# seung-lab/igneous

Hardware: NVIDIA H100
Metric: Mvoxels/s on 2048x2048x1024 uint32 seg per GPU (downsample+CCL+mesh) @1/2/4/8 H100; % HBM roofline (higher is better)
Workload: dtype u32

## Files before the change

### igneous_b200/csrc/simplify.cu

```cuda
#include <cub/device/device_radix_sort.cuh>
#include <cub/device/device_scan.cuh>

#include <stdlib.h>

#include <algorithm>
#include <type_traits>

#include "mesher.h"

namespace ign {

constexpr uint64_t S_KEYMAX = 0xFFFFFFFFFFFFFFFFull;
constexpr int S_MAXV = 32;
constexpr int S_VCAP = 64;
constexpr int VB = 11;

struct Simp {
  uint64_t U, T;
  double* pos;
  double* Q;
  uint32_t* face;
  uint32_t* flabel;
  uint8_t* falive;
  uint8_t* valive;
// ... 10 lines not shown
__device__ __forceinline__ uint32_t s_unmix(uint32_t x) {
  x ^= x >> 16; x *= 0x43021123U; x ^= x >> 15 ^ x >> 30; x *= 0x1d69e2a5U; x ^= x >> 16;
  return x;
}
__device__ __forceinline__ uint32_t s_mix16(uint32_t x) {
  x &= 0xFFFFu;
  x = (x * 0x2F35u) & 0xFFFFu; x ^= x >> 7;
  x = (x * 0x4A6Bu) & 0xFFFFu; x ^= x >> 9;
  x = (x * 0x9E37u) & 0xFFFFu; x ^= x >> 8;
  return x;
}
__device__ __forceinline__ uint32_t s_unmix16(uint32_t x) {
  x &= 0xFFFFu;
  x ^= x >> 8; x = (x * 0x7787u) & 0xFFFFu;
  x ^= x >> 9; x = (x * 0x1243u) & 0xFFFFu;
  x ^= x >> 7; x ^= x >> 14; x = (x * 0xEB1Du) & 0xFFFFu;
  return x;
}
__device__ __forceinline__ unsigned long long s_key(double cost, uint32_t h, uint32_t salt) {
  const float c = __double2float_rn(cost);
  return ((unsigned long long)__float_as_uint(c) << 32) | s_mix(h ^ salt);
}

__device__ __forceinline__ double s_qeval(const double* q, const double* p) {
  const double x = p[0], y = p[1], z = p[2];
  return q[0] * x * x + 2.0 * q[1] * x * y + 2.0 * q[2] * x * z + 2.0 * q[3] * x + q[4] * y * y +
         2.0 * q[5] * y * z + 2.0 * q[6] * y + q[7] * z * z + 2.0 * q[8] * z + q[9];
}

__device__ int s_twins(const Simp& s, uint32_t f, uint32_t u, uint32_t v, uint32_t* twin) {
  int cnt = 0;
  const uint32_t* lu = s.vf + (uint64_t)u * S_VCAP;
  const uint32_t cu = s.vn[u];
  for (uint32_t j = 0; j < cu; j++) {
    const uint32_t h = lu[j];
    const uint32_t g = h / 3;
    if (g == f || !s.falive[g]) continue;
    const uint32_t* fv = s.face + 3 * (uint64_t)g;
    if (fv[0] == v || fv[1] == v || fv[2] == v) {
      if (cnt == 0) *twin = h;
      cnt++;
    }
  }
  return cnt;
}

struct SEval {
  bool valid;
  double cost;
  uint32_t keep, remove;
  double p[3];
};

__device__ __forceinline__ void s_cost(const double* Q, const double* pos, double max_err2, uint32_t u, uint32_t v,
                                       uint64_t gu, uint64_t gv, bool bu, bool bv, SEval* e) {
  e->valid = false;
  if (bu && bv) return;
  const double* Qu = Q + 10 * gu;
  const double* Qv = Q + 10 * gv;
  double q[10];
#pragma unroll
  for (int i = 0; i < 10; i++) q[i] = Qu[i] + Qv[i];
  const double* pu = pos + 3 * gu;
  const double* pv = pos + 3 * gv;
  double best[3], cost;
  if (bu) {
    e->keep = u;
    e->remove = v;
    best[0] = pu[0]; best[1] = pu[1]; best[2] = pu[2];
    cost = s_qeval(q, best);
  } else if (bv) {
    e->keep = v;
    e->remove = u;
    best[0] = pv[0]; best[1] = pv[1]; best[2] = pv[2];
    cost = s_qeval(q, best);
  } else {
    e->keep = u < v ? u : v;
    e->remove = u < v ? v : u;
    const double* pk = u < v ? pu : pv;
    const double* pr = u < v ? pv : pu;
    const double kk[3] = {pk[0], pk[1], pk[2]}, rr[3] = {pr[0], pr[1], pr[2]};
    const double mid[3] = {(kk[0] + rr[0]) * 0.5, (kk[1] + rr[1]) * 0.5, (kk[2] + rr[2]) * 0.5};
    const double ck = s_qeval(q, kk), cr = s_qeval(q, rr), cm = s_qeval(q, mid);
    cost = ck;
    best[0] = kk[0]; best[1] = kk[1]; best[2] = kk[2];
    if (cr < cost) { cost = cr; best[0] = rr[0]; best[1] = rr[1]; best[2] = rr[2]; }
    if (cm < cost) { cost = cm; best[0] = mid[0]; best[1] = mid[1]; best[2] = mid[2]; }
  }
  if (cost < 0.0) cost = 0.0;
  if (!(cost <= max_err2)) return;
  e->valid = true;
  e->cost = cost;
  e->p[0] = best[0]; e->p[1] = best[1]; e->p[2] = best[2];
}

__global__ void __launch_bounds__(256)
    k_simp_init_verts(const uint64_t* __restrict__ vkeys, uint64_t U, double rx, double ry, double rz,
                      double* __restrict__ pos, uint8_t* __restrict__ valive,
                      uint8_t* __restrict__ vbound, uint32_t* __restrict__ vn) {
  const uint64_t i = blockIdx.x * (uint64_t)blockDim.x + threadIdx.x;
  if (i >= U) return;
  const uint64_t k = vkeys[i];
  const double x = (double)(k & ((1u << VB) - 1));
  const double y = (double)((k >> VB) & ((1u << VB) - 1));
  const double z = (double)((k >> (2 * VB)) & ((1u << VB) - 1));
  pos[3 * i + 0] = x * 0.5 * rx;
  pos[3 * i + 1] = y * 0.5 * ry;
  pos[3 * i + 2] = z * 0.5 * rz;
  valive[i] = 1;
  vbound[i] = 0;
  vn[i] = 0;
}

__global__ void __launch_bounds__(256)
    k_simp_init_faces(const uint32_t* __restrict__ faces_local, const uint32_t* __restrict__ tri_off,
                      const uint32_t* __restrict__ vert_off, uint32_t K, uint64_t T,
                      uint32_t* __restrict__ face, uint32_t* __restrict__ flabel,
                      uint8_t* __restrict__ falive, uint32_t* __restrict__ node_vertex,
                      uint32_t* __restrict__ node_id) {
  const uint64_t f = blockIdx.x * (uint64_t)blockDim.x + threadIdx.x;
  if (f >= T) return;
  uint32_t lo = 1, hi = K;
  while (lo < hi) {
    const uint32_t mid = (lo + hi + 1) >> 1;
    if (tri_off[mid] <= f) lo = mid;
    else hi = mid - 1;
  }
  flabel[f] = lo;
  falive[f] = 1;
  for (int k = 0; k < 3; k++) {
    const uint32_t g = faces_local[3 * f + k] + vert_off[lo];
    face[3 * f + k] = g;
    node_vertex[3 * f + k] = g;
    node_id[3 * f + k] = (uint32_t)(3 * f + k);
  }
}

__global__ void __launch_bounds__(256)
    k_simp_link(const uint32_t* __restrict__ sv, const uint32_t* __restrict__ sh, uint64_t n,
                uint32_t* __restrict__ vf, uint32_t* __restrict__ vn, uint32_t* overflow) {
  const uint64_t i = blockIdx.x * (uint64_t)blockDim.x + threadIdx.x;
  if (i >= n) return;
  const uint32_t v = sv[i];
  if (i > 0 && sv[i - 1] == v) return;
  uint32_t c = 0;
  for (uint64_t j = i; j < n && sv[j] == v; j++) {
// ... 109 lines not shown
__host__ __device__ inline bool sl_fits_smem(uint32_t T, uint32_t U, uint32_t threads, size_t smem_bytes,
                                             bool resumed = false) {
  const uint32_t cap = (uint32_t)SL_LIST_PER * threads;
  return 3ull * T <= 65536ull && T <= cap && U <= cap && sl_layout(T, U, resumed).need <= smem_bytes;
}
__host__ __device__ inline uint32_t sl_wcap(uint32_t T, uint32_t U, uint32_t threads, size_t smem_bytes,
                                            bool resumed, uint32_t limit) {
  const size_t w = SL_WCAP + (smem_bytes - sl_layout(T, U, resumed).need) / SL_WIN_BYTES;
  const size_t m = threads < limit ? threads : limit;
  return (uint32_t)(w < m ? w : m);
}

struct SlArgs {
  double* pos;
  double* Q;
  uint32_t* face;
  uint8_t* falive;
  uint8_t* valive;
  const uint8_t* vbound;
  float* ecost;
  unsigned long long* key1;
  uint8_t* fstate;
  uint8_t* vflag;
  uint8_t* vlose;
  uint32_t *flist, *flist2;
  uint32_t *vlist, *vlist2;
  const uint32_t* tri_off;
  const uint32_t* vert_off;
  const uint32_t* target;
  const uint32_t* order;
  uint32_t K;
  uint32_t base;
  uint32_t cls;
  uint32_t* counters;
  double max_err2;
  int max_rounds;
  uint32_t smem_bytes;
  uint32_t* mq_next;
  uint32_t smem_next;
  const uint32_t* mq;
  uint16_t* finv;
  int persist;
  uint32_t* lrec;
  uint32_t* trace;
  uint32_t wcap_max;
  uint32_t group_min;
};

constexpr int SL_HIST = 1664, SL_HP = 16, SL_HW = 64, SL_HR = S_MAXV + 2, SL_HCLS = SL_HP + SL_HW + SL_HR;

constexpr int SL_MREC = 8;
constexpr int SL_LREC = 7;
constexpr int SL_NPH = 9;

struct SlShared {
  uint32_t work, alive, progress, ncol, nwin, stop, slow, counter, npass;
  uint32_t ring8, ring16;
  uint32_t nnarrow, nwide;
  uint32_t rec, valive;
  unsigned long long visits, wins;
  long long t_label;
  uint32_t nrecost;
  uint32_t ngroup[3];
  unsigned long long ph[SL_NPH];
  long long t_prev;
};

template <bool SM>
struct SlLab {
  typedef typename std::conditional<SM, uint16_t, uint32_t>::type idx_t;
  uint32_t T, U, tbase, vbase, target, label;
  idx_t *fc0, *fc1, *fc2;
  idx_t *fmap, *vmap;
  uint32_t* gface;
  uint8_t* fstate;
  uint8_t* vflag;
  uint8_t* vlose;
  typedef typename std::conditional<SM, uint32_t, unsigned long long>::type key_t;
  key_t* key1;
  bool fmt16;
  uint32_t wcap;
  idx_t* ring;
  idx_t *flist, *flist2, *vlist, *vlist2;
};

template <bool SM>
__device__ __forceinline__ uint32_t sl_fget(const SlLab<SM>& L, uint32_t f, int c) {
  if (SM) return c == 0 ? L.fc0[f] : (c == 1 ? L.fc1[f] : L.fc2[f]);
  return L.gface[3 * (uint64_t)f + c] - L.vbase;
}
template <bool SM>
__device__ __forceinline__ void sl_fset(const SlLab<SM>& L, uint32_t f, int c, uint32_t x) {
  typedef typename SlLab<SM>::idx_t idx_t;
  if (SM) {
    if (c == 0) L.fc0[f] = (idx_t)x;
    else if (c == 1) L.fc1[f] = (idx_t)x;
    else L.fc2[f] = (idx_t)x;
  } else {
    L.gface[3 * (uint64_t)f + c] = x + L.vbase;
  }
}
template <bool SM, bool R>
__device__ __forceinline__ uint64_t sl_vg(const SlLab<SM>& L, uint32_t v) {
  return L.vbase + (uint64_t)(R ? (uint32_t)L.vmap[v] : v);
}
template <bool SM, bool R>
// ... 4 lines not shown
__device__ __forceinline__ void sl_vor(uint8_t* vflag, uint32_t v, uint32_t bits) {
  const uintptr_t a = (uintptr_t)(vflag + v);
  if ((*(volatile uint8_t*)a & bits) == bits) return;
  const uint32_t word = bits << (8 * (a & 3));
  if (SM) {
    asm volatile("red.shared.or.b32 [%0], %1;" ::"r"((uint32_t)__cvta_generic_to_shared((void*)(a & ~(uintptr_t)3))), "r"(word) : "memory");
  } else {
    atomicOr((uint32_t*)(a & ~(uintptr_t)3), word);
  }
}
template <bool SM>
__device__ __forceinline__ void sl_vclear(uint8_t* vflag, uint32_t v, uint32_t bits) {
  const uintptr_t a = (uintptr_t)(vflag + v);
  const uint32_t word = ~(bits << (8 * (a & 3)));
  if (SM) {
    asm volatile("red.shared.and.b32 [%0], %1;" ::"r"((uint32_t)__cvta_generic_to_shared((void*)(a & ~(uintptr_t)3))), "r"(word) : "memory");
  } else {
    atomicAnd((uint32_t*)(a & ~(uintptr_t)3), word);
  }
}
__device__ __forceinline__ void sl_post(unsigned long long* key1, uint32_t u, uint32_t v, unsigned long long key) {
  if (key < *(volatile unsigned long long*)&key1[u]) atomicMin(&key1[u], key);
  if (key < *(volatile unsigned long long*)&key1[v]) atomicMin(&key1[v], key);
}
__device__ __forceinline__ void sl_post(uint32_t* key1, uint32_t u, uint32_t v, uint32_t key) {
  if (key < *(volatile uint32_t*)&key1[u])
    asm volatile("red.shared.min.u32 [%0], %1;" ::"r"((uint32_t)__cvta_generic_to_shared(key1 + u)), "r"(key) : "memory");
  if (key < *(volatile uint32_t*)&key1[v])
    asm volatile("red.shared.min.u32 [%0], %1;" ::"r"((uint32_t)__cvta_generic_to_shared(key1 + v)), "r"(key) : "memory");
}
template <bool SM>
__device__ __forceinline__ typename SlLab<SM>::key_t sl_key(const SlLab<SM>& L, float cost, uint32_t hl, uint32_t salt) {
  typedef typename SlLab<SM>::key_t key_t;
  const uint32_t bits = __float_as_uint(cost);
  if (SM || L.fmt16) return (key_t)((((bits >> 15) & 0xFFFFu) << 16) | s_mix16((hl ^ salt) & 0xFFFFu));
  return (key_t)(((unsigned long long)bits << 32) | s_mix(hl ^ salt));
}
template <bool SM>
__device__ __forceinline__ uint32_t sl_key_edge(const SlLab<SM>& L, typename SlLab<SM>::key_t key, uint32_t salt) {
  if (SM || L.fmt16) return s_unmix16((uint32_t)key & 0xFFFFu) ^ (salt & 0xFFFFu);
  return s_unmix((uint32_t)((unsigned long long)key & 0xFFFFFFFFull)) ^ salt;
}

template <bool SM, bool R>
__device__ __forceinline__ void sl_cost(const SlArgs& A, const SlLab<SM>& L, uint32_t u, uint32_t v, SEval* e) {
  s_cost(A.Q, A.pos, A.max_err2, u, v, sl_vg<SM, R>(L, u), sl_vg<SM, R>(L, v), (L.vflag[u] & VF_BOUND) != 0,
         (L.vflag[v] & VF_BOUND) != 0, e);
}

template <bool SM>
__device__ __forceinline__ uint32_t sl_kcorner(const SlLab<SM>& L, uint32_t f, uint32_t k) {
  return sl_fget<SM>(L, f, 0) == k ? 0u : (sl_fget<SM>(L, f, 1) == k ? 1u : 2u);
}
template <bool SM, bool R>
__device__ __forceinline__ uint32_t sl_recost(const SlArgs& A, const SlLab<SM>& L, uint32_t f, uint32_t c) {
  const uint32_t u = sl_fget<SM>(L, f, (int)c), v = sl_fget<SM>(L, f, (int)((c + 1) % 3));
  SEval ev;
  sl_cost<SM, R>(A, L, u, v, &ev);
  if (!ev.valid) return 3;
  A.ecost[3 * (uint64_t)(L.tbase + sl_fo<SM, R>(L, f)) + c] = __double2float_rn(ev.cost);
  return 2;
}

template <bool SM, bool R>
__device__ __forceinline__ bool sl_flips(const SlArgs& A, const SlLab<SM>& L, const uint32_t* a, uint32_t w,
                                         const double* best) {
  double P[3][3], N[3][3];
#pragma unroll
  for (int k = 0; k < 3; k++) {
    const double* p = A.pos + 3 * sl_vg<SM, R>(L, a[k]);
    P[k][0] = p[0]; P[k][1] = p[1]; P[k][2] = p[2];
  }
#pragma unroll
  for (int k = 0; k < 3; k++) {
    const bool mv = (a[k] == w);
    N[k][0] = mv ? best[0] : P[k][0];
    N[k][1] = mv ? best[1] : P[k][1];
    N[k][2] = mv ? best[2] : P[k][2];
  }
  const double ax = P[1][0] - P[0][0], ay = P[1][1] - P[0][1], az = P[1][2] - P[0][2];
  const double bx = P[2][0] - P[0][0], by = P[2][1] - P[0][1], bz = P[2][2] - P[0][2];
  const double n0x = ay * bz - az * by, n0y = az * bx - ax * bz, n0z = ax * by - ay * bx;
  const double cx = N[1][0] - N[0][0], cy = N[1][1] - N[0][1], cz = N[1][2] - N[0][2];
  const double dx = N[2][0] - N[0][0], dy = N[2][1] - N[0][1], dz = N[2][2] - N[0][2];
  const double n1x = cy * dz - cz * dy, n1y = cz * dx - cx * dz, n1z = cx * dy - cy * dx;
  const double dot = n0x * n1x + n0y * n1y + n0z * n1z;
  return !(dot > 0.0);
}

__device__ __forceinline__ void sl_others(const uint32_t* a, uint32_t w, uint32_t* o1, uint32_t* o2) {
  if (a[0] == w) { *o1 = a[1]; *o2 = a[2]; }
  else if (a[1] == w) { *o1 = a[2]; *o2 = a[0]; }
  else { *o1 = a[0]; *o2 = a[1]; }
}

__device__ __forceinline__ uint32_t sl_distinct(uint32_t x1, uint32_t x2, uint32_t n, uint32_t lane, bool* f1,
                                                bool* f2) {
  const uint32_t FULL = 0xFFFFFFFFu;
  const bool have = lane < n;
  const uint32_t m1 = __match_any_sync(FULL, x1);
  const uint32_t m2 = __match_any_sync(FULL, x2);
  *f1 = have && ((int)lane == __ffs(m1) - 1);
  bool in1 = false;
  for (uint32_t j = 0; j < n; j++) in1 |= (__shfl_sync(FULL, x1, j) == x2);
  *f2 = have && ((int)lane == __ffs(m2) - 1) && !in1;
  return __popc(__ballot_sync(FULL, *f1)) + __popc(__ballot_sync(FULL, *f2));
}

template <bool SM, typename IDX, typename PRED>
__device__ __forceinline__ uint32_t sl_compact(IDX*& list, IDX*& list2, uint32_t n, uint32_t* counter, PRED alive) {
  const uint32_t FULL = 0xFFFFFFFFu;
// ... 25 lines not shown
    if (lane == 31 && inc) base = atomicAdd(counter, inc);
    base = __shfl_sync(FULL, base, 31) + inc - cnt;
#pragma unroll
    for (int k = 0; k < SL_LIST_PER; k++)
      if ((m >> k) & 1u) list[base++] = keep[k];
  } else {
    for (uint32_t i0 = (tid & ~31u); i0 < n; i0 += blockDim.x) {
      const uint32_t i = i0 + lane;
      IDX e = 0;
      bool al = false;
      if (i < n) {
        e = list[i];
        al = alive((uint32_t)e);
      }
      const uint32_t bal = __ballot_sync(FULL, al);
      if (!bal) continue;
      uint32_t base = 0;
      const int leader = __ffs(bal) - 1;
      if ((int)lane == leader) base = atomicAdd(counter, (uint32_t)__popc(bal));
      base = __shfl_sync(FULL, base, leader);
      if (al) list2[base + __popc(bal & ((1u << lane) - 1u))] = e;
    }
    IDX* t = list;
    list = list2;
    list2 = t;
  }
  __syncthreads();
  const uint32_t kept = *counter;
  __syncthreads();
  return kept;
}

#define SL_MARK(id)                                   \
  do {                                                \
    if (A.trace != nullptr && tid == 0) {             \
      const long long _t = clock64();                 \
      sh.ph[id] += (unsigned long long)(_t - sh.t_prev); \
      sh.t_prev = _t;                                 \
    }                                                 \
  } while (0)

extern __shared__ __align__(16) unsigned char sl_smem[];

__device__ __forceinline__ SlWin* sl_win() { return (SlWin*)sl_smem; }

__device__ __forceinline__ uint32_t sl_width(uint32_t nfu, uint32_t nfv, uint32_t wmin) {
  const uint32_t n = nfu > nfv ? nfu : nfv;
  const uint32_t w = n <= 8u ? 8u : (n <= 16u ? 16u : 32u);
  return w > wmin ? w : wmin;
}

template <bool SM, bool R, int W>
__device__ __forceinline__ void sl_group_pass(const SlArgs& A, const SlLab<SM>& L, SlShared& sh, uint32_t first,
                                              uint32_t last, uint32_t* nev) {
  static_assert(W == 8 || W == 16 || W == 32, "group width");
  const uint32_t FULL = 0xFFFFFFFFu;
  const uint32_t tid = threadIdx.x, lane = tid & 31u, warp = tid >> 5, NW = blockDim.x >> 5;
  constexpr uint32_t G = 32 / W;
  const uint32_t gl = lane & (W - 1), goff = lane & ~(uint32_t)(W - 1);
  const uint32_t wmask = W == 32 ? FULL : (1u << W) - 1u;
  const uint32_t gmask = wmask << goff;
  const uint32_t gidx = lane / W;
  SlWin* const win = sl_win();
  for (uint32_t base = first + warp * G; base < last; base += NW * G) {
    bool act = base + gidx < last;
    uint32_t slot = 0, nfu = 0, nfv = 0;
    if (act) {
      slot = win[base + gidx].order;
      nfu = win[slot].cnt[0]; nfv = win[slot].cnt[1];
    }
    act = act && sl_width(nfu, nfv, A.group_min) == (uint32_t)W;
    const uint32_t b_act = __ballot_sync(FULL, act && gl == 0);
    if (!b_act) continue;
    if (lane == 0) atomicAdd(&sh.ngroup[W == 8 ? 0 : (W == 16 ? 1 : 2)], (uint32_t)__popc(b_act));
    if (W == 32 && act && gl == 0 && (nfu > (uint32_t)S_MAXV || nfv > (uint32_t)S_MAXV)) atomicAdd(&A.counters[25], 1u);
    uint32_t fu = 0, fv = 0, u = 0, v = 0, hl = 0, k = 0;
    bool ok = false;
    if (act) {
      if (gl < nfu) fu = L.ring[(2 * slot) * S_MAXV + gl];
      if (gl < nfv) fv = L.ring[(2 * slot + 1) * S_MAXV + gl];
      u = win[slot].u; v = win[slot].v; hl = win[slot].h; k = win[slot].keep;
      ok = !(win[slot].flags & WF_BAD) && nfu <= (uint32_t)S_MAXV && nfv <= (uint32_t)S_MAXV;
    }
    uint32_t au[3] = {0, 0, 0}, av[3] = {0, 0, 0};
    if (ok && gl < nfu) { au[0] = sl_fget<SM>(L, fu, 0); au[1] = sl_fget<SM>(L, fu, 1); au[2] = sl_fget<SM>(L, fu, 2); }
    if (ok && gl < nfv) { av[0] = sl_fget<SM>(L, fv, 0); av[1] = sl_fget<SM>(L, fv, 1); av[2] = sl_fget<SM>(L, fv, 2); }
    {
      bool flip = false;
      if (ok && gl < nfu && au[0] != v && au[1] != v && au[2] != v) flip = sl_flips<SM, R>(A, L, au, u, win[slot].best);
      if (ok && gl < nfv && av[0] != u && av[1] != u && av[2] != u) flip |= sl_flips<SM, R>(A, L, av, v, win[slot].best);
      if (__ballot_sync(FULL, flip) & gmask) ok = false;
    }
    const uint32_t rm = (k == u) ? v : u;
    const uint64_t gk = sl_vg<SM, R>(L, k), gr = sl_vg<SM, R>(L, rm);
    double* Qk = A.Q + 10 * gk;
    const double* Qr = A.Q + 10 * gr;
    double qk = 0.0, qr = 0.0, qk2 = 0.0, qr2 = 0.0;
    if (ok && gl < 10) { qk = Qk[gl]; qr = Qr[gl]; }
    if (W == 8 && ok && gl < 2) { qk2 = Qk[gl + 8]; qr2 = Qr[gl + 8]; }
    const bool hu = ok && gl < nfu, hv = ok && gl < nfv;
    uint32_t x1 = 0xF0000000u + lane, x2 = 0xF1000000u + lane, y1 = 0xF2000000u + lane, y2 = 0xF3000000u + lane;
    if (hu) sl_others(au, u, &x1, &x2);
    if (hv) sl_others(av, v, &y1, &y2);
    const uint32_t nu = ok ? nfu : 0u, nv = ok ? nfv : 0u;
    uint32_t nmax = nu > nv ? nu : nv;
#pragma unroll
    for (uint32_t d = W; d < 32u; d <<= 1) {
      const uint32_t o = __shfl_xor_sync(FULL, nmax, d);
      nmax = o > nmax ? o : nmax;
    }
    const uint32_t mu1 = __match_any_sync(FULL, x1) & gmask, mu2 = __match_any_sync(FULL, x2) & gmask;
    const uint32_t mv1 = __match_any_sync(FULL, y1) & gmask, mv2 = __match_any_sync(FULL, y2) & gmask;
    bool inu = false, inv = false, c1 = false, c2 = false;
    for (uint32_t j = 0; j < nmax; j++) {
      const uint32_t sx1 = __shfl_sync(FULL, x1, j, W), sy1 = __shfl_sync(FULL, y1, j, W), sy2 = __shfl_sync(FULL, y2, j, W);
      if (j < nu) inu |= (sx1 == x2);
      if (j < nv) {
        inv |= (sy1 == y2);
        c1 |= (x1 == sy1) | (x1 == sy2);
        c2 |= (x2 == sy1) | (x2 == sy2);
      }
    }
    const bool f1 = hu && ((int)lane == __ffs(mu1) - 1);
    const bool f2 = hu && ((int)lane == __ffs(mu2) - 1) && !inu;
    const bool g1 = hv && ((int)lane == __ffs(mv1) - 1);
    const bool g2 = hv && ((int)lane == __ffs(mv2) - 1) && !inv;
    const uint32_t b_f1 = __ballot_sync(FULL, f1), b_f2 = __ballot_sync(FULL, f2);
    const uint32_t b_g1 = __ballot_sync(FULL, g1), b_g2 = __ballot_sync(FULL, g2);
    const uint32_t b_c1 = __ballot_sync(FULL, f1 && c1), b_c2 = __ballot_sync(FULL, f2 && c2);
    const uint32_t b_sh = __ballot_sync(FULL, hu && (x1 == v || x2 == v));
    const uint32_t nnu = __popc(b_f1 & gmask) + __popc(b_f2 & gmask), nnv = __popc(b_g1 & gmask) + __popc(b_g2 & gmask);
    const uint32_t common = __popc(b_c1 & gmask) + __popc(b_c2 & gmask), shared = __popc(b_sh & gmask);
    const bool go = ok && nnu <= (uint32_t)S_MAXV && nnv <= (uint32_t)S_MAXV && shared == 2 && common == 2;
    if (act && !go && gl == 0) {
      const uint32_t f = hl / 3, c = hl - 3 * f;
      const uint32_t st = L.fstate[f];
      L.fstate[f] = (uint8_t)((st & ~(3u << (2 * c))) | (1u << (2 * c)));
      sl_vclear<SM>(L.vflag, u, VF_END);
      sl_vclear<SM>(L.vflag, v, VF_END);
      atomicOr(&sh.progress, 1u);
    }
    const bool rm_is_u = (rm == u);
    const bool hr = go && (rm_is_u ? hu : hv);
    const uint32_t rf = rm_is_u ? fu : fv;
    const uint32_t r0 = rm_is_u ? au[0] : av[0], r1 = rm_is_u ? au[1] : av[1], r2 = rm_is_u ? au[2] : av[2];
    const bool dies = hr && (r0 == k || r1 == k || r2 == k);
    if (hr) {
      if (dies) L.fstate[rf] = (uint8_t)(L.fstate[rf] & 0x7Fu);
      else sl_fset<SM>(L, rf, r0 == rm ? 0 : (r1 == rm ? 1 : 2), k);
    }
    const uint32_t dead = __popc(__ballot_sync(FULL, dies) & gmask);
    if (go) {
      if (hu && x1 != v && x2 != v) { sl_vor<SM>(L.vflag, x1, VF_RDIRTY); sl_vor<SM>(L.vflag, x2, VF_RDIRTY); }
      if (hv && y1 != u && y2 != u) { sl_vor<SM>(L.vflag, y1, VF_RDIRTY); sl_vor<SM>(L.vflag, y2, VF_RDIRTY); }
      if (gl < 10) Qk[gl] = qk + qr;
      if (gl >= 10 && gl < 13) A.pos[3 * gk + (gl - 10)] = win[slot].best[gl - 10];
      if (W == 8) {
        if (gl < 2) Qk[gl + 8] = qk2 + qr2;
        else if (gl < 5) A.pos[3 * gk + (gl - 2)] = win[slot].best[gl - 2];
      }
      if (gl == 0) {
        sl_vclear<SM>(L.vflag, k, VF_END);
        sl_vclear<SM>(L.vflag, rm, 0xFFu);
        atomicSub(&sh.alive, dead);
        atomicAdd(&sh.ncol, 1u);
        atomicOr(&sh.progress, 1u);
      }
    }
    __syncwarp();
    uint32_t m = 0, ck = 0, st0 = 0, st1 = 0;
    if (go && gl < nfu) {
      st0 = L.fstate[fu];
      if (st0 & 0x80u) {
        const uint32_t c = sl_kcorner<SM>(L, fu, k);
        ck = c;
        m |= (k < sl_fget<SM>(L, fu, (int)((c + 1) % 3)) ? 1u : 0u) | (sl_fget<SM>(L, fu, (int)((c + 2) % 3)) < k ? 2u : 0u);
      }
    }
    if (go && gl < nfv) {
      st1 = L.fstate[fv];
      if (st1 & 0x80u) {
        const uint32_t c = sl_kcorner<SM>(L, fv, k);
        ck |= c << 2;
        m |= (k < sl_fget<SM>(L, fv, (int)((c + 1) % 3)) ? 4u : 0u) | (sl_fget<SM>(L, fv, (int)((c + 2) % 3)) < k ? 8u : 0u);
      }
    }
    const uint32_t cnt = __popc(m);
    uint32_t inc = cnt;
#pragma unroll
    for (uint32_t d = 1; d < W; d <<= 1) {
      const uint32_t o = __shfl_up_sync(FULL, inc, d, W);
      if (gl >= d) inc += o;
    }
    const uint32_t P = inc - cnt, N = __shfl_sync(FULL, inc, W - 1, W);
    uint32_t rounds = (N + W - 1) / W;
#pragma unroll
    for (uint32_t d = W; d < 32u; d <<= 1) {
      const uint32_t o = __shfl_xor_sync(FULL, rounds, d);
      rounds = o > rounds ? o : rounds;
    }
    uint32_t res = 0;
    for (uint32_t r = 0; r < rounds; r++) {
      const uint32_t idx = r * W + gl;
      uint32_t own = 0;
      for (uint32_t j = 1; j < W; j++)
        if (__shfl_sync(FULL, P, j, W) <= idx) own = j;
      const uint32_t mo = __shfl_sync(FULL, m, own, W), po = __shfl_sync(FULL, P, own, W);
      const uint32_t fuo = __shfl_sync(FULL, fu, own, W), fvo = __shfl_sync(FULL, fv, own, W);
      const uint32_t cko = __shfl_sync(FULL, ck, own, W);
      if (idx < N) {
        uint32_t b = mo;
        for (uint32_t q = idx - po; q; q--) b &= b - 1;
        const uint32_t bit = (uint32_t)__ffs(b) - 1, side = bit >> 1;
        const uint32_t c = (((cko >> (2 * side)) & 3u) + 2u * (bit & 1u)) % 3u;
        res |= sl_recost<SM, R>(A, L, side ? fvo : fuo, c) << (2 * r);
        (*nev)++;
      }
    }
    uint32_t q = P;
#pragma unroll
    for (uint32_t bit = 0; bit < 4; bit++) {
      const uint32_t val = __shfl_sync(FULL, res, q % W, W);
      if ((m >> bit) & 1u) {
        const uint32_t side = bit >> 1, es = (val >> (2 * (q / W))) & 3u;
        const uint32_t c = (((ck >> (2 * side)) & 3u) + 2u * (bit & 1u)) % 3u;
        if (side) st1 = (st1 & ~(3u << (2 * c))) | (es << (2 * c));
        else st0 = (st0 & ~(3u << (2 * c))) | (es << (2 * c));
        q++;
      }
    }
    if (m & 3u) L.fstate[fu] = (uint8_t)st0;
    if (m & 12u) L.fstate[fv] = (uint8_t)st1;
  }
}

template <bool R>
__device__ void sl_migrate(const SlArgs& A, const SlLab<true>& L, SlShared& sh, const uint16_t* flist, uint32_t nF,
                           int r) {
  const uint32_t FULL = 0xFFFFFFFFu;
  const uint32_t tid = threadIdx.x, NT = blockDim.x, lane = tid & 31u, warp = tid >> 5, NW = NT >> 5;
  uint32_t* const wsum = (uint32_t*)sl_win();
  const uint32_t per = (L.U + NT - 1) / NT, v0 = min(tid * per, L.U), v1 = min(v0 + per, L.U);
  uint32_t cnt = 0;
  for (uint32_t v = v0; v < v1; v++) cnt += L.vflag[v] & VF_ALIVE;
  uint32_t inc = cnt;
#pragma unroll
  for (int d = 1; d < 32; d <<= 1) {
    const uint32_t o = __shfl_up_sync(FULL, inc, d);
    if ((int)lane >= d) inc += o;
  }
  if (lane == 31) wsum[warp] = inc;
  __syncthreads();
  if (warp == 0) {
    const uint32_t t = lane < NW ? wsum[lane] : 0u;
    uint32_t x = t;
#pragma unroll
    for (int d = 1; d < 32; d <<= 1) {
      const uint32_t o = __shfl_up_sync(FULL, x, d);
      if ((int)lane >= d) x += o;
    }
    if (lane < NW) wsum[lane] = x - t;
  }
  __syncthreads();
  uint32_t j = wsum[warp] + inc - cnt;
  for (uint32_t v = v0; v < v1; v++) {
    const uint32_t fl = L.vflag[v];
    if (!(fl & VF_ALIVE)) continue;
    A.vlist[L.vbase + j] = (uint32_t)(R ? L.vmap[v] : v) | (fl << 16);
    L.key1[v] = j++;
  }
// ... 236 lines not shown
        if (!split || tid >= nbt) {
          const uint32_t first = split ? tid - nbt : tid, step = split ? NT - nbt : NT;
          for (uint32_t i = first; i < nF; i += 2 * step) {
            const uint32_t i2 = i + step;
            const bool two = i2 < nF;
            const uint32_t fa = flist[i], fb = two ? (uint32_t)flist[i2] : fa;
            const bool la = (L.fstate[fa] & 0x80u) != 0, lb = two && (L.fstate[fb] & 0x80u) != 0;
            uint32_t x[6] = {0, 0, 0, 0, 0, 0}, fl[6] = {0, 0, 0, 0, 0, 0};
            if (la) { x[0] = sl_fget<SM>(L, fa, 0); x[1] = sl_fget<SM>(L, fa, 1); x[2] = sl_fget<SM>(L, fa, 2); }
            if (lb) { x[3] = sl_fget<SM>(L, fb, 0); x[4] = sl_fget<SM>(L, fb, 1); x[5] = sl_fget<SM>(L, fb, 2); }
            if (la) { fl[0] = L.vflag[x[0]]; fl[1] = L.vflag[x[1]]; fl[2] = L.vflag[x[2]]; }
            if (lb) { fl[3] = L.vflag[x[3]]; fl[4] = L.vflag[x[4]]; fl[5] = L.vflag[x[5]]; }
#pragma unroll
            for (int c = 0; c < 6; c++) {
              if (!(fl[c] & VF_END)) continue;
              const uint32_t sl = (uint32_t)L.key1[x[c]];
              const uint32_t p = atomicAdd(&win[sl >> 1].cnt[sl & 1u], 1u);
              if (p < (uint32_t)S_MAXV) L.ring[sl * S_MAXV + p] = (idx_t)(c < 3 ? fa : fb);
              if (p == 8u) sh.ring8 = 1;
              if (p == 16u) sh.ring16 = 1;
            }
          }
        }
      }
      __syncthreads();
      SL_MARK(5);
      SL_MARK(6);
      if (A.trace != nullptr) {
        for (uint32_t i = tid; i < 2 * nb; i += NT) {
          const uint32_t n = win[i >> 1].cnt[i & 1u];
          atomicAdd(&A.trace[SL_HIST + SL_HCLS * A.cls + SL_HP + SL_HW + (n <= (uint32_t)S_MAXV ? n : S_MAXV + 1)], 1u);
        }
      }
      for (uint32_t i0 = warp * 32; i0 < nb; i0 += NT) {
        const uint32_t i = i0 + lane;
        const bool have = i < nb;
        const bool narrow = have && sl_width(win[i].cnt[0], win[i].cnt[1], A.group_min) == 8u;
        const uint32_t bn = __ballot_sync(FULL, narrow), bw = __ballot_sync(FULL, have && !narrow);
        uint32_t pn = 0, pw = 0;
        if (lane == 0) {
          if (bn) pn = atomicAdd(&sh.nnarrow, (uint32_t)__popc(bn));
          if (bw) pw = atomicAdd(&sh.nwide, (uint32_t)__popc(bw));
        }
        pn = __shfl_sync(FULL, pn, 0);
        pw = __shfl_sync(FULL, pw, 0);
        const uint32_t below = (1u << lane) - 1u;
        if (narrow) win[pn + __popc(bn & below)].order = i;
        else if (have) win[nb - 1 - (pw + __popc(bw & below))].order = i;
      }
      __syncthreads();
      {
        uint32_t nev = 0;
        const uint32_t wmin = A.group_min, n8 = sh.nnarrow;
        if (n8) sl_group_pass<SM, R, 8>(A, L, sh, 0, n8, &nev);
        if (wmin == 16u || (wmin == 8u && sh.ring8)) sl_group_pass<SM, R, 16>(A, L, sh, n8, nb, &nev);
        if (wmin == 32u || sh.ring16) sl_group_pass<SM, R, 32>(A, L, sh, n8, nb, &nev);
        if (nev) atomicAdd(&sh.nrecost, nev);
      }
      __syncthreads();
      SL_MARK(7);
      if (total <= L.wcap) break;
    }
    if (tid == 0) {
      const uint32_t passes = sh.npass;
      if (passes > 1) atomicAdd(&A.counters[24], 1u);
      if (A.trace != nullptr) atomicAdd(&A.trace[SL_HIST + SL_HCLS * A.cls + (passes < (uint32_t)SL_HP ? passes : SL_HP) - 1], 1u);
    }
    if (tid == 0 && A.trace != nullptr && sh.rec == 0 && r < 400) {
      A.trace[4 * r + 0] = sh.progress;
      A.trace[4 * r + 1] = sh.ncol;
      A.trace[4 * r + 2] = sh.alive;
      A.trace[4 * r + 3] = nF;
    }
    if (A.trace != nullptr && tid == 0) sh.visits += nF;
    if (tid == 0) {
      sh.valive -= sh.ncol;
      uint32_t stop = 0;
      if (!sh.progress) {
        stop = 1;
      } else {
        if ((uint64_t)sh.ncol * 1000 < (uint64_t)sh.alive) sh.slow++;
        else sh.slow = 0;
        if (sh.slow >= 4) stop = 1;
      }
      sh.stop = stop;
    }
    __syncthreads();
    SL_MARK(8);
    if (sh.stop) {
      r++;
      break;
    }
    if (r & 1) {
      nF = sl_compact<SM>(flist, flist2, nF, &sh.counter, [&](uint32_t f) { return (L.fstate[f] & 0x80u) != 0; });
      if (!SM) nV = sl_compact<SM>(vlist, vlist2, nV, &sh.counter, [&](uint32_t v) { return (L.vflag[v] & VF_ALIVE) != 0; });
      if (SM && A.mq_next != nullptr && sl_fits_smem(nF, sh.valive, NT / 2, A.smem_next, true)) {
        if constexpr (SM) sl_migrate<R>(A, L, sh, flist, nF, r);
        migrated = true;
        r++;
        break;
      }
    }
  }
  for (uint32_t f = tid; f < T; f += NT) {
    const bool al = L.fstate[f] & 0x80u;
    const uint32_t fo = sl_fo<SM, R>(L, f);
    if (migrated && al) continue;
    A.falive[L.tbase + fo] = al ? 1 : 0;
    if (SM && al) {
// ... 383 lines not shown
      }
      if (c == 0 && ev_full && err == cudaSuccess) err = cudaEventRecord(ev_full, cs[0]);
    }
    for (int c = 1; c < SL_NCLASS && err == cudaSuccess; c++) {
      if (resume[c]) {
        const uint32_t nt = (uint32_t)SL_CLASS_THREADS[c];
        err = cudaStreamWaitEvent(cs[c], c == 1 ? ev_full : ev[c - 1], 0);
        if (err != cudaSuccess) break;
        A.cls = (uint32_t)c;
        A.smem_bytes = (uint32_t)sl_dyn[c];
        A.smem_next = c + 1 < SL_NCLASS ? (uint32_t)sl_dyn[c + 1] : 0u;
        A.mq_next = (c + 1 < SL_NCLASS) ? d_mq + (size_t)SL_MREC * K * c : nullptr;
        A.mq = d_mq + (size_t)SL_MREC * K * (c - 1);
        const uint64_t slots = (uint64_t)ctx->sm_count * (1024 / nt);
        const unsigned grid = A.persist ? (unsigned)(resume[c] < slots ? resume[c] : slots) : resume[c];
        k_simp_resume<<<grid, nt, sl_dyn[c], cs[c]>>>(A);
        ctx->launches++;
        err = cudaGetLastError();
      }
      if (ev[c] && err == cudaSuccess) err = cudaEventRecord(ev[c], cs[c]);
    }
    for (int c = 1; c < SL_NCLASS && err == cudaSuccess; c++)
      if (ev[c]) err = cudaStreamWaitEvent(ctx->stream, ev[c], 0);
    if (ev_full) cudaEventDestroy(ev_full);
    for (int c = 0; c < SL_NCLASS; c++) {
      if (ev[c]) cudaEventDestroy(ev[c]);
      if (c > 0 && cs[c]) cudaStreamDestroy(cs[c]);
    }
    prof_end(ctx, slot);
    IGN_CUDA(err);
  }

  uint32_t* fscan = node_v;
  uint32_t* fflag = node_h;
  size_t tb = tmpb;
  IGN_LAUNCH(ctx, k_simp_flags_u32, blocks_for(U, 256), 256, 0, s.valive, U, vflag32);
  IGN_CUDA(cub::DeviceScan::ExclusiveSum(tmp, tb, vflag32, vscan, (int)U, ctx->stream));
  IGN_LAUNCH(ctx, k_simp_flags_u32, blocks_for(T, 256), 256, 0, s.falive, T, fflag);
  tb = tmpb;
  IGN_CUDA(cub::DeviceScan::ExclusiveSum(tmp, tb, fflag, fscan, (int)T, ctx->stream));
  ctx->launches += 4;
  uint32_t last[4], hflags[32];
  IGN_TRY(small_d2h(ctx, &last[0], vscan + (U - 1), 4));
  IGN_TRY(small_d2h(ctx, &last[1], vflag32 + (U - 1), 4));
  IGN_TRY(small_d2h(ctx, &last[2], fscan + (T - 1), 4));
  IGN_TRY(small_d2h(ctx, &last[3], fflag + (T - 1), 4));
  IGN_TRY(small_d2h(ctx, hflags, flags, sizeof(hflags)));
  IGN_TRY(small_sync(ctx));
  if (hflags[12] != 0) {
    set_error("simplify: a vertex has more than %d incident faces", S_VCAP);
    return IGN_ERR_UNSUPPORTED;
  }
  if (A.trace) {
    std::vector<uint32_t> tr(1600);
    IGN_CUDA(cudaMemcpy(tr.data(), A.trace, 1600 * 4, cudaMemcpyDeviceToHost));
    unsigned long long phs[SL_NPH];
    IGN_CUDA(cudaMemcpy(phs, A.trace + 1600, sizeof(phs), cudaMemcpyDeviceToHost));
    static const char* names[SL_NPH] = {"P1", "P2 keys", "P3 lose", "P4 select", "setup", "E1 rings", "E2a cost", "E2 validate+collapse+recost", "stop+compact"};
    unsigned long long tot = 0;
    for (int q = 0; q < SL_NPH; q++) tot += phs[q];
    for (int q = 0; q < SL_NPH; q++)
      fprintf(stderr, "phase %-27s %6.2f %%  %10.3f Mcycles\n", names[q], 100.0 * phs[q] / (tot ? tot : 1), phs[q] / 1e6);
    fprintf(stderr, "cost evaluations: %u initial (k_simp_ecost), %u after collapses (E2), %u half-edges without a cost in P2\n",
            hflags[26], hflags[27], hflags[28]);
    fprintf(stderr, "winners by E2 group width: %u of 8 lanes, %u of 16, %u of 32\n", hflags[29], hflags[30], hflags[31]);
    {
      std::vector<uint32_t> rec(SL_LREC * (size_t)K);
      IGN_CUDA(cudaMemcpy(rec.data(), A.lrec, rec.size() * 4, cudaMemcpyDeviceToHost));
      static const uint32_t edges[] = {0, 500, 1000, 2000, 3000, 4000, 6000, 8000, 10000, 12000, 16000, 32000, 64000, 0xFFFFFFFFu};
      const int nedges = (int)(sizeof(edges) / sizeof(edges[0]));
      for (int c = 0; c < SL_NCLASS; c++) {
        int per_sm = 0;
        IGN_CUDA(cudaOccupancyMaxActiveBlocksPerMultiprocessor(&per_sm, k_simp_labels, SL_CLASS_THREADS[c], sl_dyn[c]));
        fprintf(stderr, "size class %d: %4d threads, %6zu B dynamic shared memory, %d CTAs per SM, %u labels\n", c,
                SL_CLASS_THREADS[c], sl_dyn[c], per_sm, ccount[c]);
      }
      fprintf(stderr, "%7s %12s %7s %8s %10s %10s %10s %9s %9s  class(sm/hy/gl)\n", "threads", "faces<", "labels", "rounds", "Mcycles", "SM Mcyc", "Mvisits", "kwins", "cyc/round");
      double sr = 0, sv = 0, sc = 0, srr = 0, svv = 0, srv = 0, src = 0, svc = 0;
      uint64_t sm_total[SL_NCLASS] = {0, 0, 0};
      for (int szc = 0; szc < SL_NCLASS; szc++) {
        for (int b = 0; b + 1 < nedges; b++) {
          uint64_t n = 0, rounds = 0, kc = 0, ksm = 0, vis = 0, wins = 0, cls[4] = {0, 0, 0, 0};
          for (uint64_t i = 0; i < K; i++) {
            const uint32_t* q = &rec[SL_LREC * i];
            if (q[1] == 0 || (int)(q[5] >> 2) != szc || q[0] < edges[b] || q[0] >= edges[b + 1]) continue;
            n++; rounds += q[1]; kc += q[2]; ksm += q[6]; vis += q[3]; wins += q[4]; cls[q[5] & 3]++;
            const double R = q[1], V = q[3], C = q[2] * 1024.0;
            sr += R; sv += V; sc += C; srr += R * R; svv += V * V; srv += R * V; src += R * C; svc += V * C;
          }
          sm_total[szc] += ksm;
          if (n) fprintf(stderr, "%7d %12u %7llu %8.1f %10.2f %10.2f %10.3f %9.1f %9.0f  %llu/%llu/%llu\n", SL_CLASS_THREADS[szc], edges[b + 1],
                         (unsigned long long)n, (double)rounds / n, kc * 1024.0 / 1e6, ksm * 1024.0 / 1e6, vis / 1e6, wins / 1e3,
                         rounds ? kc * 1024.0 / rounds : 0.0, (unsigned long long)cls[1], (unsigned long long)cls[2],
                         (unsigned long long)cls[3]);
        }
      }
      fprintf(stderr, "SM Mcycles by starting class: %.0f + %.0f + %.0f = %.0f; labels resumed in the 512- / 256-thread class: %u / %u\n",
              sm_total[0] * 1024.0 / 1e6, sm_total[1] * 1024.0 / 1e6, sm_total[2] * 1024.0 / 1e6,
              (sm_total[0] + sm_total[1] + sm_total[2]) * 1024.0 / 1e6, hflags[17], hflags[18]);
      std::vector<uint32_t> hist(SL_NCLASS * SL_HCLS);
      IGN_CUDA(cudaMemcpy(hist.data(), A.trace + SL_HIST, hist.size() * 4, cudaMemcpyDeviceToHost));
      for (int c = 0; c < SL_NCLASS; c++) {
        const uint32_t* h = &hist[SL_HCLS * c];
        fprintf(stderr, "class %d passes/round (1..%d+):", SL_CLASS_THREADS[c], SL_HP);
        for (int b = 0; b < SL_HP; b++) fprintf(stderr, " %u", h[b]);
        fprintf(stderr, "\nclass %d winners/round (bins of 16, last %d+):", SL_CLASS_THREADS[c], 16 * (SL_HW - 1));
        for (int b = 0; b < SL_HW; b++) fprintf(stderr, " %u", h[SL_HP + b]);
        fprintf(stderr, "\nclass %d ring length per winner side (0..%d, more):", SL_CLASS_THREADS[c], S_MAXV);
        for (int b = 0; b < SL_HR; b++) fprintf(stderr, " %u", h[SL_HP + SL_HW + b]);
        fprintf(stderr, "\n");
      }
      const double det = srr * svv - srv * srv;
      if (det != 0) fprintf(stderr, "fit: cycles ~= %.0f * rounds + %.2f * face visits   (totals: %.0f rounds, %.3g visits, %.3g cycles)\n",
                            (src * svv - svc * srv) / det, (svc * srr - src * srv) / det, sr, sv, sc);
    }
    for (int r = 0; r < 400 && getenv("IGN_SIMP_TRACE_ROUNDS") && (tr[4 * r + 2] || tr[4 * r + 3]); r++)
      fprintf(stderr, "gpu round %d progress %u collapses %u alive %u list %u\n", r, tr[4 * r], tr[4 * r + 1], tr[4 * r + 2], tr[4 * r + 3]);
  }
// ... 69 lines not shown
```

Baseline: 6095.

## Reuse merged quadric and keep position from registers when recosting edges after collapse

Recosting after a collapse now reuses the merged quadric of the kept vertex. It broadcasts that quadric across the lane group with shuffles and takes the kept vertex's new position from the window, so only the other endpoint's Q and position are loaded from global memory. The group passes also rotate their starting warp to balance work across the 8/16/32-wide passes, and the replaced-corner index and dies test now reuse values already in registers. A trace-only flip-rejection counter is added. The shuffle now runs for inactive lanes too, which adds some instructions.

```diff
diff --git a/igneous_b200/csrc/simplify.cu b/igneous_b200/csrc/simplify.cu
--- a/igneous_b200/csrc/simplify.cu
+++ b/igneous_b200/csrc/simplify.cu
@@ -86,17 +86,10 @@
   double p[3];
 };
 
-__device__ __forceinline__ void s_cost(const double* Q, const double* pos, double max_err2, uint32_t u, uint32_t v,
-                                       uint64_t gu, uint64_t gv, bool bu, bool bv, SEval* e) {
+__device__ __forceinline__ void s_cost_q(const double* q, const double* pu, const double* pv, double max_err2,
+                                         uint32_t u, uint32_t v, bool bu, bool bv, SEval* e) {
   e->valid = false;
   if (bu && bv) return;
-  const double* Qu = Q + 10 * gu;
-  const double* Qv = Q + 10 * gv;
-  double q[10];
-#pragma unroll
-  for (int i = 0; i < 10; i++) q[i] = Qu[i] + Qv[i];
-  const double* pu = pos + 3 * gu;
-  const double* pv = pos + 3 * gv;
   double best[3], cost;
   if (bu) {
     e->keep = u;
@@ -111,9 +104,9 @@
   } else {
     e->keep = u < v ? u : v;
     e->remove = u < v ? v : u;
-    const double* pk = u < v ? pu : pv;
-    const double* pr = u < v ? pv : pu;
-    const double kk[3] = {pk[0], pk[1], pk[2]}, rr[3] = {pr[0], pr[1], pr[2]};
+    const bool uk = u < v;
+    const double kk[3] = {uk ? pu[0] : pv[0], uk ? pu[1] : pv[1], uk ? pu[2] : pv[2]};
+    const double rr[3] = {uk ? pv[0] : pu[0], uk ? pv[1] : pu[1], uk ? pv[2] : pu[2]};
     const double mid[3] = {(kk[0] + rr[0]) * 0.5, (kk[1] + rr[1]) * 0.5, (kk[2] + rr[2]) * 0.5};
     const double ck = s_qeval(q, kk), cr = s_qeval(q, rr), cm = s_qeval(q, mid);
     cost = ck;
@@ -126,6 +119,18 @@
   e->valid = true;
   e->cost = cost;
   e->p[0] = best[0]; e->p[1] = best[1]; e->p[2] = best[2];
+}
+
+__device__ __forceinline__ void s_cost(const double* Q, const double* pos, double max_err2, uint32_t u, uint32_t v,
+                                       uint64_t gu, uint64_t gv, bool bu, bool bv, SEval* e) {
+  e->valid = false;
+  if (bu && bv) return;
+  const double* Qu = Q + 10 * gu;
+  const double* Qv = Q + 10 * gv;
+  double q[10];
+#pragma unroll
+  for (int i = 0; i < 10; i++) q[i] = Qu[i] + Qv[i];
+  s_cost_q(q, pos + 3 * gu, pos + 3 * gv, max_err2, u, v, bu, bv, e);
 }
 
 __global__ void __launch_bounds__(256)
@@ -341,6 +346,7 @@
 constexpr int SL_MREC = 8;
 constexpr int SL_LREC = 7;
 constexpr int SL_NPH = 9;
+constexpr int SL_TFLIP = 1620;
 
 struct SlShared {
   uint32_t work, alive, progress, ncol, nwin, stop, slow, counter, npass;
@@ -451,11 +457,30 @@
 __device__ __forceinline__ uint32_t sl_kcorner(const SlLab<SM>& L, uint32_t f, uint32_t k) {
   return sl_fget<SM>(L, f, 0) == k ? 0u : (sl_fget<SM>(L, f, 1) == k ? 1u : 2u);
 }
-template <bool SM, bool R>
-__device__ __forceinline__ uint32_t sl_recost(const SlArgs& A, const SlLab<SM>& L, uint32_t f, uint32_t c) {
-  const uint32_t u = sl_fget<SM>(L, f, (int)c), v = sl_fget<SM>(L, f, (int)((c + 1) % 3));
+template <bool SM, bool R, int W>
+__device__ __forceinline__ uint32_t sl_recost_k(const SlArgs& A, const SlLab<SM>& L, bool has, uint32_t f,
+                                                uint32_t c, uint32_t k, double qs, double qs2, const double* pk) {
+  uint32_t u = k, v = k;
+  if (has) { u = sl_fget<SM>(L, f, (int)c); v = sl_fget<SM>(L, f, (int)((c + 1) % 3)); }
+  const bool ku = (u == k);
+  const uint64_t go = sl_vg<SM, R>(L, ku ? v : u);
+  double q[10], po[3] = {0.0, 0.0, 0.0};
+#pragma unroll
+  for (int i = 0; i < 10; i++) q[i] = has ? A.Q[10 * go + i] : 0.0;
+  if (has) { po[0] = A.pos[3 * go]; po[1] = A.pos[3 * go + 1]; po[2] = A.pos[3 * go + 2]; }
+#pragma unroll
+  for (int i = 0; i < 10; i++)
+    q[i] += __shfl_sync(0xFFFFFFFFu, (W == 8 && i >= 8) ? qs2 : qs, (W == 8 && i >= 8) ? i - 8 : i, W);
+  if (!has) return 0;
+  double pu[3], pv[3];
+#pragma unroll
+  for (int i = 0; i < 3; i++) {
+    const double b = pk[i];
+    pu[i] = ku ? b : po[i];
+    pv[i] = ku ? po[i] : b;
+  }
   SEval ev;
-  sl_cost<SM, R>(A, L, u, v, &ev);
+  s_cost_q(q, pu, pv, A.max_err2, u, v, (L.vflag[u] & VF_BOUND) != 0, (L.vflag[v] & VF_BOUND) != 0, &ev);
   if (!ev.valid) return 3;
   A.ecost[3 * (uint64_t)(L.tbase + sl_fo<SM, R>(L, f)) + c] = __double2float_rn(ev.cost);
   return 2;
@@ -587,7 +612,7 @@
 
 template <bool SM, bool R, int W>
 __device__ __forceinline__ void sl_group_pass(const SlArgs& A, const SlLab<SM>& L, SlShared& sh, uint32_t first,
-                                              uint32_t last, uint32_t* nev) {
+                                              uint32_t last, uint32_t w0, uint32_t* nev) {
   static_assert(W == 8 || W == 16 || W == 32, "group width");
   const uint32_t FULL = 0xFFFFFFFFu;
   const uint32_t tid = threadIdx.x, lane = tid & 31u, warp = tid >> 5, NW = blockDim.x >> 5;
@@ -597,7 +622,7 @@
   const uint32_t gmask = wmask << goff;
   const uint32_t gidx = lane / W;
   SlWin* const win = sl_win();
-  for (uint32_t base = first + warp * G; base < last; base += NW * G) {
+  for (uint32_t base = first + ((warp + NW - w0) % NW) * G; base < last; base += NW * G) {
     bool act = base + gidx < last;
     uint32_t slot = 0, nfu = 0, nfv = 0;
     if (act) {
@@ -609,22 +634,24 @@
     if (!b_act) continue;
     if (lane == 0) atomicAdd(&sh.ngroup[W == 8 ? 0 : (W == 16 ? 1 : 2)], (uint32_t)__popc(b_act));
     if (W == 32 && act && gl == 0 && (nfu > (uint32_t)S_MAXV || nfv > (uint32_t)S_MAXV)) atomicAdd(&A.counters[25], 1u);
-    uint32_t fu = 0, fv = 0, u = 0, v = 0, hl = 0, k = 0;
+    uint32_t fu = 0, fv = 0, u = 0, v = 0, k = 0;
     bool ok = false;
     if (act) {
       if (gl < nfu) fu = L.ring[(2 * slot) * S_MAXV + gl];
       if (gl < nfv) fv = L.ring[(2 * slot + 1) * S_MAXV + gl];
-      u = win[slot].u; v = win[slot].v; hl = win[slot].h; k = win[slot].keep;
+      u = win[slot].u; v = win[slot].v; k = win[slot].keep;
       ok = !(win[slot].flags & WF_BAD) && nfu <= (uint32_t)S_MAXV && nfv <= (uint32_t)S_MAXV;
     }
     uint32_t au[3] = {0, 0, 0}, av[3] = {0, 0, 0};
     if (ok && gl < nfu) { au[0] = sl_fget<SM>(L, fu, 0); au[1] = sl_fget<SM>(L, fu, 1); au[2] = sl_fget<SM>(L, fu, 2); }
     if (ok && gl < nfv) { av[0] = sl_fget<SM>(L, fv, 0); av[1] = sl_fget<SM>(L, fv, 1); av[2] = sl_fget<SM>(L, fv, 2); }
-    {
-      bool flip = false;
-      if (ok && gl < nfu && au[0] != v && au[1] != v && au[2] != v) flip = sl_flips<SM, R>(A, L, au, u, win[slot].best);
-      if (ok && gl < nfv && av[0] != u && av[1] != u && av[2] != u) flip |= sl_flips<SM, R>(A, L, av, v, win[slot].best);
-      if (__ballot_sync(FULL, flip) & gmask) ok = false;
+    uint32_t flip = 0;
+    if (ok && gl < nfu && au[0] != v && au[1] != v && au[2] != v && sl_flips<SM, R>(A, L, au, u, win[slot].best)) flip = 1u;
+    if (ok && gl < nfv && av[0] != u && av[1] != u && av[2] != u && sl_flips<SM, R>(A, L, av, v, win[slot].best)) flip |= 2u;
+    if (__ballot_sync(FULL, flip != 0) & gmask) ok = false;
+    if (A.trace != nullptr) {
+      const uint32_t b_u = __ballot_sync(FULL, flip & 1u) & gmask, b_v = __ballot_sync(FULL, flip & 2u) & gmask;
+      if (act && gl == 0 && (b_u || b_v)) atomicAdd(&A.trace[SL_TFLIP + (b_u && b_v ? 2 : (b_u ? 0 : 1))], 1u);
     }
     const uint32_t rm = (k == u) ? v : u;
     const uint64_t gk = sl_vg<SM, R>(L, k), gr = sl_vg<SM, R>(L, rm);
@@ -637,6 +664,8 @@
     uint32_t x1 = 0xF0000000u + lane, x2 = 0xF1000000u + lane, y1 = 0xF2000000u + lane, y2 = 0xF3000000u + lane;
     if (hu) sl_others(au, u, &x1, &x2);
     if (hv) sl_others(av, v, &y1, &y2);
+    const bool rm_is_u = (rm == u);
+    const uint32_t crm = rm_is_u ? (au[0] == u ? 0u : (au[1] == u ? 1u : 2u)) : (av[0] == v ? 0u : (av[1] == v ? 1u : 2u));
     const uint32_t nu = ok ? nfu : 0u, nv = ok ? nfv : 0u;
     uint32_t nmax = nu > nv ? nu : nv;
 #pragma unroll
@@ -668,30 +697,29 @@
     const uint32_t common = __popc(b_c1 & gmask) + __popc(b_c2 & gmask), shared = __popc(b_sh & gmask);
     const bool go = ok && nnu <= (uint32_t)S_MAXV && nnv <= (uint32_t)S_MAXV && shared == 2 && common == 2;
     if (act && !go && gl == 0) {
-      const uint32_t f = hl / 3, c = hl - 3 * f;
+      const uint32_t hl = win[slot].h, f = hl / 3, c = hl - 3 * f;
       const uint32_t st = L.fstate[f];
       L.fstate[f] = (uint8_t)((st & ~(3u << (2 * c))) | (1u << (2 * c)));
       sl_vclear<SM>(L.vflag, u, VF_END);
       sl_vclear<SM>(L.vflag, v, VF_END);
       atomicOr(&sh.progress, 1u);
     }
-    const bool rm_is_u = (rm == u);
     const bool hr = go && (rm_is_u ? hu : hv);
     const uint32_t rf = rm_is_u ? fu : fv;
-    const uint32_t r0 = rm_is_u ? au[0] : av[0], r1 = rm_is_u ? au[1] : av[1], r2 = rm_is_u ? au[2] : av[2];
-    const bool dies = hr && (r0 == k || r1 == k || r2 == k);
+    const bool dies = hr && (rm_is_u ? (x1 == k || x2 == k) : (y1 == k || y2 == k));
     if (hr) {
       if (dies) L.fstate[rf] = (uint8_t)(L.fstate[rf] & 0x7Fu);
-      else sl_fset<SM>(L, rf, r0 == rm ? 0 : (r1 == rm ? 1 : 2), k);
+      else sl_fset<SM>(L, rf, (int)crm, k);
     }
     const uint32_t dead = __popc(__ballot_sync(FULL, dies) & gmask);
+    const double qs = qk + qr, qs2 = qk2 + qr2;
     if (go) {
       if (hu && x1 != v && x2 != v) { sl_vor<SM>(L.vflag, x1, VF_RDIRTY); sl_vor<SM>(L.vflag, x2, VF_RDIRTY); }
       if (hv && y1 != u && y2 != u) { sl_vor<SM>(L.vflag, y1, VF_RDIRTY); sl_vor<SM>(L.vflag, y2, VF_RDIRTY); }
-      if (gl < 10) Qk[gl] = qk + qr;
+      if (gl < 10) Qk[gl] = qs;
       if (gl >= 10 && gl < 13) A.pos[3 * gk + (gl - 10)] = win[slot].best[gl - 10];
       if (W == 8) {
-        if (gl < 2) Qk[gl + 8] = qk2 + qr2;
+        if (gl < 2) Qk[gl + 8] = qs2;
         else if (gl < 5) A.pos[3 * gk + (gl - 2)] = win[slot].best[gl - 2];
       }
       if (gl == 0) {
@@ -743,14 +771,17 @@
       const uint32_t mo = __shfl_sync(FULL, m, own, W), po = __shfl_sync(FULL, P, own, W);
       const uint32_t fuo = __shfl_sync(FULL, fu, own, W), fvo = __shfl_sync(FULL, fv, own, W);
       const uint32_t cko = __shfl_sync(FULL, ck, own, W);
-      if (idx < N) {
+      const bool has = idx < N;
+      uint32_t f = 0, c = 0;
+      if (has) {
         uint32_t b = mo;
         for (uint32_t q = idx - po; q; q--) b &= b - 1;
         const uint32_t bit = (uint32_t)__ffs(b) - 1, side = bit >> 1;
-        const uint32_t c = (((cko >> (2 * side)) & 3u) + 2u * (bit & 1u)) % 3u;
-        res |= sl_recost<SM, R>(A, L, side ? fvo : fuo, c) << (2 * r);
+        c = (((cko >> (2 * side)) & 3u) + 2u * (bit & 1u)) % 3u;
+        f = side ? fvo : fuo;
         (*nev)++;
       }
+      res |= sl_recost_k<SM, R, W>(A, L, has, f, c, k, qs, qs2, win[slot].best) << (2 * r);
     }
     uint32_t q = P;
 #pragma unroll
@@ -1093,9 +1124,16 @@
       {
         uint32_t nev = 0;
         const uint32_t wmin = A.group_min, n8 = sh.nnarrow;
-        if (n8) sl_group_pass<SM, R, 8>(A, L, sh, 0, n8, &nev);
-        if (wmin == 16u || (wmin == 8u && sh.ring8)) sl_group_pass<SM, R, 16>(A, L, sh, n8, nb, &nev);
-        if (wmin == 32u || sh.ring16) sl_group_pass<SM, R, 32>(A, L, sh, n8, nb, &nev);
+        uint32_t w0 = 0;
+        if (n8) {
+          sl_group_pass<SM, R, 8>(A, L, sh, 0, n8, w0, &nev);
+          w0 = (w0 + (n8 + 3u) / 4u) % NW;
+        }
+        if (wmin == 16u || (wmin == 8u && sh.ring8)) {
+          sl_group_pass<SM, R, 16>(A, L, sh, n8, nb, w0, &nev);
+          w0 = (w0 + (nb - n8 + 1u) / 2u) % NW;
+        }
+        if (wmin == 32u || sh.ring16) sl_group_pass<SM, R, 32>(A, L, sh, n8, nb, w0, &nev);
         if (nev) atomicAdd(&sh.nrecost, nev);
       }
       __syncthreads();
@@ -1585,8 +1623,8 @@
     return IGN_ERR_UNSUPPORTED;
   }
   if (A.trace) {
-    std::vector<uint32_t> tr(1600);
-    IGN_CUDA(cudaMemcpy(tr.data(), A.trace, 1600 * 4, cudaMemcpyDeviceToHost));
+    std::vector<uint32_t> tr(SL_HIST);
+    IGN_CUDA(cudaMemcpy(tr.data(), A.trace, SL_HIST * 4, cudaMemcpyDeviceToHost));
     unsigned long long phs[SL_NPH];
     IGN_CUDA(cudaMemcpy(phs, A.trace + 1600, sizeof(phs), cudaMemcpyDeviceToHost));
     static const char* names[SL_NPH] = {"P1", "P2 keys", "P3 lose", "P4 select", "setup", "E1 rings", "E2a cost", "E2 validate+collapse+recost", "stop+compact"};
@@ -1597,6 +1635,8 @@
     fprintf(stderr, "cost evaluations: %u initial (k_simp_ecost), %u after collapses (E2), %u half-edges without a cost in P2\n",
             hflags[26], hflags[27], hflags[28]);
     fprintf(stderr, "winners by E2 group width: %u of 8 lanes, %u of 16, %u of 32\n", hflags[29], hflags[30], hflags[31]);
+    fprintf(stderr, "winners rejected by E2 flip tests: %u on the u side only, %u on the v side only, %u on both\n",
+            tr[SL_TFLIP], tr[SL_TFLIP + 1], tr[SL_TFLIP + 2]);
     {
       std::vector<uint32_t> rec(SL_LREC * (size_t)K);
       IGN_CUDA(cudaMemcpy(rec.data(), A.lrec, rec.size() * 4, cudaMemcpyDeviceToHost));
```

Measured after the change: 6300, median of 6. 1.03x the previous value.
